# QData/FastSK

Measured on AMD Instinct MI355X. Metric: gkm kernel build: mismatch-combos/s, higher is better.
Workload: dtype u4 count planes (v_dot8_u32_u4), u32 register sums, u64 triangle (plain stores on the first pass over reset rows, else atomics); 1 GPU; config5: synthetic DNA 100000 x 300 bp, g=12 m=8 exact, 495 combos; n_seq=100000, seq_len=300, g=12, m=8, combos=495, parallelism=single GPU

## Files before the change

fastsk_amd/csrc/fsk_bytesel.h:

```cpp
#pragma once
#include "fsk_platform.h"

namespace fsk_hw {

template <int B>
__device__ __forceinline__ uint32_t add_byte(uint32_t acc, uint32_t packed) {
    static_assert(B >= 0 && B < 4, "a dword has four bytes");
#ifdef FSK_EMU
    return acc + ((packed >> (8 * B)) & 255u);
#else
    uint32_t d;
    if constexpr (B == 0)
        asm volatile("v_add_u32_sdwa %0, %1, %2 dst_sel:DWORD dst_unused:UNUSED_PAD src0_sel:BYTE_0 src1_sel:DWORD" : "=v"(d) : "v"(packed), "v"(acc));
    else if constexpr (B == 1)
        asm volatile("v_add_u32_sdwa %0, %1, %2 dst_sel:DWORD dst_unused:UNUSED_PAD src0_sel:BYTE_1 src1_sel:DWORD" : "=v"(d) : "v"(packed), "v"(acc));
    else if constexpr (B == 2)
        asm volatile("v_add_u32_sdwa %0, %1, %2 dst_sel:DWORD dst_unused:UNUSED_PAD src0_sel:BYTE_2 src1_sel:DWORD" : "=v"(d) : "v"(packed), "v"(acc));
    else
        asm volatile("v_add_u32_sdwa %0, %1, %2 dst_sel:DWORD dst_unused:UNUSED_PAD src0_sel:BYTE_3 src1_sel:DWORD" : "=v"(d) : "v"(packed), "v"(acc));
    return d;
#endif
}

template <int W>
__device__ __forceinline__ uint32_t xor_word(uint32_t packed, uint32_t x) {
    static_assert(W == 0 || W == 1, "a dword has two halves");
#ifdef FSK_EMU
    return ((packed >> (16 * W)) & 0xffffu) ^ x;
#else
    uint32_t d;
    if constexpr (W == 0)
        asm("v_xor_b32_sdwa %0, %1, %2 dst_sel:DWORD dst_unused:UNUSED_PAD src0_sel:WORD_0 src1_sel:DWORD" : "=v"(d) : "v"(packed), "v"(x));
    else
        asm("v_xor_b32_sdwa %0, %1, %2 dst_sel:DWORD dst_unused:UNUSED_PAD src0_sel:WORD_1 src1_sel:DWORD" : "=v"(d) : "v"(packed), "v"(x));
    return d;
#endif
}

__device__ __forceinline__ void first_use(uint32_t& a, uint32_t& b, uint32_t& c, uint32_t& d, uint32_t& e, uint32_t& f, uint32_t& g, uint32_t& h) {
#ifndef FSK_EMU
    asm volatile("" : "+v"(a), "+v"(b), "+v"(c), "+v"(d), "+v"(e), "+v"(f), "+v"(g), "+v"(h) : : "memory");
#endif
}

}
```

fastsk_amd/csrc/fsk_engine_dense_shift.hip:

```cpp
#include "fsk_engine_internal.h"
#include "fsk_kernels_dense_shift.h"

#include <map>

using namespace fsk_detail;

namespace fsk {

#define FSK_DMA_SHIFT 1
#define FSK_DMA_KERNEL k_dense_tile_shift
#define FSK_DMA_COMPACT 0
#include "fsk_tile_kernel_dma.inc"
#undef FSK_DMA_KERNEL
#undef FSK_DMA_SHIFT

#define FSK_DMA_SHIFT 2
#define FSK_DMA_KERNEL k_dense_tile_shift_all
#include "fsk_tile_kernel_dma.inc"
#undef FSK_DMA_KERNEL
#undef FSK_DMA_COMPACT
#undef FSK_DMA_SHIFT

}

// ... 27 lines not shown
        p.n_bases = (uint32_t)chains.size();
        p.order.resize((size_t)n);
        uint32_t derived = p.n_bases;
        size_t group_begin = 0;
        for (size_t c = 0; c < chains.size(); ++c) {
            const std::vector<int>& ch = chains[c];
            const uint32_t len = (uint32_t)ch.size();
            p.order[c] = ch[0];
            if (c == 0 || chains[c - 1].size() != ch.size() || (u64)(c - group_begin) >= by_overflow) {
                p.groups.push_back(0u);
                p.groups.push_back(len);
                group_begin = c;
            }
            p.groups[p.groups.size() - 2] = (uint32_t)c + 1u;
            uint32_t lower = (uint32_t)c;
            for (uint32_t u = 1; u < len; ++u) {
                const uint32_t upper = derived++;
                p.order[upper] = ch[u];
                p.steps.push_back(upper << 16 | lower);
                p.steps.push_back(len - u);
                p.wsum += len - u;
                lower = upper;
            }
        }
        bool falling = true;
        for (size_t gi = 2; gi + 1 < p.groups.size(); gi += 2) falling = falling && p.groups[gi + 1] < p.groups[gi - 1];
        if (falling) {
            for (size_t gi = 0; gi + 1 < p.groups.size(); gi += 2) {
                p.group_steps.push_back(p.groups[gi]);
                p.group_steps.push_back(p.groups[gi + 1] - (gi + 3 < p.groups.size() ? p.groups[gi + 3] : 0u));
            }
            p.group_steps.push_back(0xffffffffu);
            p.group_steps.push_back(0u);
        }
    }
    return !p.steps.empty() && n <= 32768 && ((u64)2 * e->maxW + 32) * p.wsum < ((u64)1 << 31);
}

static void dense_shift_unpack_flags(std::vector<uint32_t>& steps, uint32_t n_bases, bool batch) {
    const size_t n_steps = steps.size() / 2;
    uint32_t r = 0, bound = 0;
    for (size_t s = 0; s < n_steps; ++s) {
        r = (steps[2 * s] & 0xffffu) < n_bases ? 0u : r + 1u;
        const uint32_t add = 30u * (r + 1u);
        if (s > 0 && (!batch || bound + add > 255u)) {
            steps[2 * s - 1] |= 256u;
            bound = 0;
        }
        bound += add;
    }
    if (n_steps > 0) steps[2 * n_steps - 1] |= 256u;
}

int dense_shift_edge_keys(fsk_engine* e, const uint8_t* chunk_pos, uint32_t panels_pad) {
    ShiftPlan& p = e->shift;
    const uint32_t n_steps = (uint32_t)(p.steps.size() / 2), np_seq = panels_pad * fsk::PANEL;
    std::vector<uint32_t> steps = p.steps;
    dense_shift_unpack_flags(steps, p.n_bases, e->tune.dense_shift_batch != 0);
    FSK_HIP(e->d_shift_steps.reserve(p.steps.size() + p.group_steps.size()));
    FSK_HIP(e->d_edge_keys.reserve((size_t)n_steps * np_seq));
    FSK_HIP(hipMemcpyAsync(e->d_shift_steps.p, steps.data(), steps.size() * sizeof(uint32_t), hipMemcpyHostToDevice, e->stream));
    if (!p.group_steps.empty())
        FSK_HIP(hipMemcpyAsync(e->d_shift_steps.p + p.steps.size(), p.group_steps.data(), p.group_steps.size() * sizeof(uint32_t), hipMemcpyHostToDevice,
                               e->stream));
    FSK_LAUNCH(fsk::k_dense_edge_keys, dim3(panels_pad, (n_steps + 3u) / 4u), dim3(256), 0, e->stream, e->view(), e->cfg.g, e->k, e->sigma, chunk_pos,
               (const uint32_t*)e->d_shift_steps.p, n_steps, np_seq, e->d_edge_keys.p);
    FSK_HIP(hipStreamSynchronize(e->stream));
    e->st.launches += 1;
    return FSK_OK;
}

int dense_shift_keymajor(fsk_engine* e, uint32_t panels_pad, int nb, uint32_t Vq8) {
    const ShiftPlan& p = e->shift;
    e->ld.shift_packed = false;
    if (e->tune.dense_shift_packed < 0 || p.max_chain != SHIFT_PACKED_CHAIN) return FSK_OK;
    const size_t plane = (size_t)panels_pad * Vq8 * fsk::PANEL * (size_t)nb;
    const size_t n_keys = (p.steps.size() / 2) * (size_t)panels_pad * fsk::PANEL;
    const size_t want = (2 * plane + n_keys) * sizeof(uint32_t);
    const char* why = nullptr;
    if (e->tune.dense_shift_plane_kb > 0 && want > (size_t)e->tune.dense_shift_plane_kb * 1024) why = "over the dense_shift_plane_kb cap";
    const size_t grow = (std::max(plane, e->d_KM.cap) - e->d_KM.cap + std::max(plane, e->d_KMH.cap) - e->d_KMH.cap +
                         std::max(n_keys, e->d_edge_offs.cap) - e->d_edge_offs.cap) * sizeof(uint32_t);
    if (!why && grow > 0) {
        size_t free_b = 0, total_b = 0;
        if (hipMemGetInfo(&free_b, &total_b) != hipSuccess) free_b = 0;
        if (grow > free_b / 2) why = "more than half of the free device memory";
        else if (e->d_KM.reserve(plane) != hipSuccess || e->d_KMH.reserve(plane) != hipSuccess || e->d_edge_offs.reserve(n_keys) != hipSuccess) {
            (void)hipGetLastError();
            e->d_KM.release(); e->d_KMH.release(); e->d_edge_offs.release();
            why = "hipMalloc failed";
        }
    }
    if (why) {
        if (e->trace())
            fprintf(stderr, "[fsk] dense shift classes: the key-major planes (%.1f MB) do not fit, %s: k_dense_shift_fix runs the corrections\n",
                    (double)want / 1e6, why);
        return FSK_OK;
    }
    const uint32_t n_pairs = panels_pad / 2u;
    const uint32_t kgrid = (uint32_t)(((size_t)n_pairs * nb * Vq8 * 16u + 255u) / 256u);
    FSK_LAUNCH(fsk::k_dense_keymajor, dim3(kgrid), dim3(256), 0, e->stream, (const uint32_t*)e->d_C4.p, n_pairs, nb, Vq8, e->d_KM.p);
    FSK_LAUNCH(fsk::k_dense_keymajor, dim3(kgrid), dim3(256), 0, e->stream, (const uint32_t*)e->d_C4H.p, n_pairs, nb, Vq8, e->d_KMH.p);
    FSK_LAUNCH(fsk::k_dense_edge_offs, dim3((uint32_t)((n_keys + 255u) / 256u)), dim3(256), 0, e->stream, (const uint16_t*)e->d_edge_keys.p, n_keys,
               e->d_edge_offs.p);
    e->st.launches += 3;
    e->ld.shift_packed = true;
    return FSK_OK;
}

int dense_shift_tiles(fsk_engine* e, u64 n_tiles, int nb, uint32_t Vq8, uint32_t nst, u64* K, int store, uint32_t panels_pad) {
    const ShiftPlan& p = e->shift;
    const bool one_launch = !p.group_steps.empty() && (e->tune.dense_shift_one_launch > 0 ||
                                                       (e->tune.dense_shift_one_launch == 0 && e->tune.tile_splits == 0 && n_tiles >= 16384));
    int base_launches = 1;
    if (one_launch) {
        FSK_LAUNCH(fsk::k_dense_tile_shift_all, dim3((uint32_t)n_tiles, 1), dim3(256), 0, e->stream, (const uint32_t*)e->d_C4.p,
                   (const uint32_t*)e->d_C4H.p, (const uint32_t*)e->d_rowmask.p, (const uint32_t*)e->d_tiletab.p, nb, Vq8, nst, (uint32_t)e->N, K,
                   (int)p.n_bases, store, (const uint32_t*)e->d_shift_steps.p + p.steps.size());
    } else {
        base_launches = (int)(p.groups.size() / 2);
        int slot0 = 0;
        for (size_t gi = 0; gi + 1 < p.groups.size(); gi += 2) {
            const int end = (int)p.groups[gi];
            FSK_LAUNCH(fsk::k_dense_tile_shift, dim3((uint32_t)n_tiles, 1), dim3(256), 0, e->stream, (const uint32_t*)e->d_C4.p,
                       (const uint32_t*)e->d_C4H.p, (const uint32_t*)e->d_rowmask.p, (const uint32_t*)e->d_tiletab.p, nb, Vq8, nst, (uint32_t)e->N, K,
                       end - slot0, gi == 0 ? store : 0, slot0, p.groups[gi + 1]);
            slot0 = end;
        }
    }
    if (e->ld.shift_packed) {
        const auto k_packed = e->tune.dense_shift_inplace != 0 ? fsk::k_dense_shift_packed<true> : fsk::k_dense_shift_packed<false>;
        FSK_LAUNCH(k_packed, dim3((uint32_t)n_tiles), dim3(256), 0, e->stream, (const uint32_t*)e->d_KM.p, (const uint32_t*)e->d_KMH.p,
                   (const uint32_t*)e->d_rowmask.p, (const uint32_t*)e->d_tiletab.p, (const uint32_t*)e->d_shift_steps.p, (uint32_t)(p.steps.size() / 2),
                   (const uint32_t*)e->d_edge_offs.p, panels_pad * fsk::PANEL, nb, Vq8, p.n_bases, (uint32_t)(30u * p.wsum), (uint32_t)e->N, K);
    } else {
        FSK_LAUNCH(fsk::k_dense_shift_fix, dim3((uint32_t)n_tiles), dim3(512), 0, e->stream, (const uint32_t*)e->d_C4.p, (const uint32_t*)e->d_C4H.p,
                   (const uint32_t*)e->d_rowmask.p, (const uint32_t*)e->d_tiletab.p, (const uint32_t*)e->d_shift_steps.p, (uint32_t)(p.steps.size() / 2),
                   (const uint16_t*)e->d_edge_keys.p, panels_pad * fsk::PANEL, nb, Vq8, (uint32_t)e->N, K);
    }
    e->st.launches += (int32_t)base_launches;
    return FSK_OK;
}

}
```

fastsk_amd/csrc/fsk_engine_internal.h:

```cpp
#pragma once
#include "fsk_common.h"

#include <algorithm>
#include <chrono>
#include <cmath>
#include <cstdarg>
#include <cstdio>
#include <cstdlib>
#include <cstring>
#include <string>
#include <array>
#include <atomic>
#include <thread>
#include <vector>

#include <cstdint>
#include <climits>

#include "../../include/fastsk_amd.h"
#include <condition_variable>
#include <functional>
#include <memory>
#include <mutex>

// ... 50 lines not shown
        cap = 0;
    }
};

template <typename H, hipError_t (*Create)(H*, unsigned), hipError_t (*Destroy)(H)>
struct Handle {
    H h = nullptr;
    Handle() = default;
    Handle(Handle&& o) noexcept : h(o.h) { o.h = nullptr; }
    Handle& operator=(Handle&& o) noexcept { std::swap(h, o.h); return *this; }
    ~Handle() { if (h) (void)Destroy(h); }
    hipError_t create(unsigned flags) { return h ? hipSuccess : Create(&h, flags); }
    operator H() const { return h; }
};
using Stream = Handle<hipStream_t, hipStreamCreateWithFlags, hipStreamDestroy>;
using Event = Handle<hipEvent_t, hipEventCreateWithFlags, hipEventDestroy>;

struct DeviceScope {
    int prev = -1, dev;
    hipError_t err = hipSuccess;
    explicit DeviceScope(int d) : dev(d) {
        if (hipGetDevice(&prev) != hipSuccess) prev = -1;
        if (prev != dev) err = hipSetDevice(dev);
    }
    ~DeviceScope() {
        if (prev >= 0 && prev != dev) (void)hipSetDevice(prev);
    }
    DeviceScope(const DeviceScope&) = delete;
    DeviceScope& operator=(const DeviceScope&) = delete;
};
#define FSK_ON_DEVICE(e)                                                                      \
    DeviceScope fsk_on_device_((e)->cfg.device);                                             \
    if (fsk_on_device_.err != hipSuccess)                                                    \
        return (e)->fail(FSK_EDEVICE, "hipSetDevice(%d) failed: %s", (e)->cfg.device, hipGetErrorString(fsk_on_device_.err))

}

using fsk_detail::DevBuf;
using fsk_detail::PinnedBuf;
using fsk_detail::Stream;
using fsk_detail::Event;

#define FSK_TUNING_KEYS(X)                                                                                                          \
    X(trace, 0, 0, 1, "stderr: the tuning in force, where the host time of a load and of a variance-mode call goes")                 \
    X(profile, -1, -1, 2, "fsk_config.profile from here on (-1: as the engine was created)")                                          \
    X(compact, -1, -1, 1, "dense: key compaction off / on whatever the alphabet says (-1: a rare symbol decides)")                   \
    X(compact_rare, -1, -1, 1, "dense: keys that occur from the places of the rare symbols (1) or a marking pass over every window (0)") \
    X(tile_splits, 0, 0, 4096, "dense: combo splits per tile (0: by the size of the launch)")                                        \
    X(dense_small, 0, 0, 1, "dense: 1 = a split tile launch (small N) leaves its sums as 32-bit staging blocks that k_dense_widen adds into K (0: one 64-bit atomic a cell and split — measured faster: the atomics drain under other workgroups' dot products)")                                        \
    X(dense_shift, 0, -1, 1, "dense: one weighted Gram product per chain of shifted combinations, the other members by edge lookups (fsk_engine_dense_shift.hip) — 1 = whenever the call is eligible, -1 = never (0: when eligible, tile_splits = 0 and the launch has 16384 tiles or more, the size from which a tile has one workgroup anyway)") \
    X(dense_shift_packed, 0, -1, 0, "dense, shift classes: the derived steps from key-major planes, eight cells an LDS read (k_dense_keymajor, k_dense_shift_packed; chains cut at nine members) — 0 = whenever the shift path runs and the planes fit, -1 = never: k_dense_shift_fix on the count panels") \
    X(dense_shift_inplace, 1, 0, 1, "dense, shift classes: k_dense_shift_packed stages a chain's first planes and makes every further step's in LDS, one nibble up and one down a sequence (a step that meets a count above 15 in its tile, and the step behind it, are staged) — 0 = every step staged") \
    X(dense_shift_batch, 1, 0, 1, "dense, shift classes: k_dense_shift_packed adds the prefix sums of several steps byte to byte and hands the bytes to its int32 sums once a batch, where the step table says so (a step at chain position r counts 30 (r + 1) against a byte's 255; a batch may span chains) — 0 = after every step") \
    X(dense_shift_one_launch, 0, -1, 1, "dense, shift classes: every chain-length group of the base products in ONE launch that flushes at the group ends without clearing (k_dense_tile_shift_all) — 1 = whenever the shift path runs, -1 = never: one k_dense_tile_shift launch a group (0: where the shift path runs by its own default rule, tile_splits = 0 and 16384 tiles or more)") \
    X(dense_shift_plane_kb, 0, 0, (int64_t)1 << 40, "dense, shift classes: the key-major planes and offsets may take this many KiB at most (0: half of the free memory; tests: the planes do not fit)") \
    X(dense_chunk, 0, 0, 1 << 24, "dense: cap of the count kernel's staging chunk, in windows (0: none)")                             \
    X(variance_dense_slots, 1, 0, 1, "variance mode, dense: 0 = zero fill + k_welford per iteration instead of storing slot triangles") \
    X(var_slots16, 1, 0, 1, "variance mode, sparse: 0 = u32 slot triangles from the start")                                          \
    X(sparse_global, 0, 0, 1, "sparse: every += as a 64-bit atomicAdd (k_sx_emit<DIRECT>) whatever N is")                             \
    X(sparse_unpacked, 0, 0, 1, "sparse: entries in the general 8 + 4 (+ 4) byte format whatever N is")                               \
    X(sparse_pairs, 1, 0, 1, "sparse: 0 = every update word 32 bits wide (1: unit products of clean runs travel two to a word)")      \
    X(sparse_sync, 0, 0, 1, "sparse: wait for every batch's word count and size its stream exactly")                                 \
    X(sparse_hint, 1, 0, 1, "sparse: 0 = the words per record of the previous set of sequences are never kept as a hint")             \
    X(sparse_exact_lanes, 0, 0, 2, "sparse: the batches of an exact accumulate never (1) / always (2) in two lanes (0: from six batches on)") \
    X(sparse_batch_records, 0, 0, (int64_t)1 << 31, "sparse: records per batch at most (0: 2^27)")                                   \
    X(guard_cap, 0, 0, (int64_t)1 << 40, "sparse: pretend the stream buffer holds this many words (0: its real size)")                \
    X(list_max_words, 0, 0, (int64_t)1 << 31, "sparse: update words of one batch beyond which its pairs go to K with atomics (0: 2^31)") \
    X(seg_scan_chunked, 0, 0, 1, "sparse: the three-launch segment scan whatever the tile count")                                    \
    X(extract_slots, 0, 0, 4, "sparse: slots per k_sx_extract_win workgroup, 1 or 4 (0: by the size of the launch)")                  \
    X(sparse_form, 0, 0, 3, "sparse: the update stage — 1 = owner bands whenever they exist, 2 = two-level blocks, 3 = 64-bit atomics (0: bands up to four LDS rounds a band, blocks beyond)") \
    X(blocks_sub_shift, 14, 4, 14, "sparse, blocks: log2 of the cells one k_sxb_consume workgroup sums in LDS (tests: small blocks on small inputs)") \
    X(blocks_max_bands, 512, 2, 512, "sparse, blocks: bands of one pass at most (tests: several passes on small inputs)")            \
    X(blocks_band_shift_max, 23, 4, 23, "sparse, blocks: log2 of a band's cells at most (tests)")                                    \
    X(blocks_pass_words, 0, 0, (int64_t)1 << 32, "sparse, blocks: update words of one pass at most (0: 2^31)")                       \
    X(sparse_desc, 0, -1, 1, "sparse, owner bands and two-level blocks: entries of many partners leave k_sx_emit as descriptors (one an entry; blocks: one per sub-band its partners fall into) that k_sx_consume / k_sxb_consume expand in LDS — 1 = always, -1 = never (0: once a batch of these sequences has shown sparse_desc_from pairs per record)") \
    X(sparse_desc_blocks, 1, 0, 1, "sparse, two-level blocks: 0 = never descriptors there (1: as sparse_desc says — one record per sub-band an entry's partners fall into)") \
    X(sparse_desc_cols, 1, 0, 3, "sparse, descriptors: where the partners are read from — 0 = the entries themselves; 1 = a column array (sequence id | multiplicity, 4 bytes) beside 8-byte entries, the entries themselves when they are packed (measured: 2-byte columns beside packed entries are no faster, 0.88 against 0.84 s in the large-g regime; 4-byte columns beside 8-byte entries 4.69 -> 4.44 ms a combo at N = 100k); tests: 2 = 4-byte columns always, 3 = 2-byte columns when N < 32768") \
    X(sparse_desc_min, 16, 1, 48, "sparse, descriptors: entries of more partners than this become descriptors (48: everything k_sx_emit does not bin in LDS; measured, large-g regime: 48 0.92 s, 32 0.85, 16 0.83-0.85, 8 0.88, 4 0.90)") \
    X(sparse_desc_from, 12, 1, 1 << 20, "sparse, descriptors: the pairs per sort record of a batch from which on the following batches use them (sparse_desc = 0)") \
    X(sparse_parts_target, 0, 0, 1 << 30, "sparse, owner bands: words of one k_sx_consume part (0: four LDS rounds' worth at least, 1/1024 of the batch's words; tests: several parts a band on small inputs)") \
    X(sparse_desc_parts, 2048, 1, 1 << 16, "sparse, descriptors: parts (k_sx_consume workgroups) the bands' streams are cut into, about") \
    X(sparse_share, 0, -1, 254, "sparse: leading kept positions sorted once per group of consecutive combos that share them (0: by cost; -1: never); batches of more than 16 slots only (smaller ones read their positions by id), and never when the presort's scratch passes a quarter of the free memory") \
    X(seed_splitmix, 0, 0, 1, "approx modes: 1 = fsk_set_seed draws the engine's older splitmix64 Fisher-Yates order (0: the reference's std::shuffle of minstd_rand0)") \
    X(mismatch_order, 0, 0, 1, "mismatch-weighted mode: 1 = the levels run from m = d down to 0 (0: from 0 up to d)")                   \
    X(collective, 0, 0, 2, "fsk_create_multi: FSK_COLL_* when fsk_config.collective is FSK_COLL_AUTO")                                \
    X(deadline_ms, 120000, -1, 86400000, "fsk_create_multi: the fail-fast bound when fsk_config.deadline_ms is 0 (negative: none)")   \
    X(svm_wg_max, 8192, 0, 8192, "fsk_svm_train: up to this many training rows the solver is one workgroup with alpha, G and y in LDS (k_svm_wg); beyond, two launches an iteration (k_svm_select_i / k_svm_select_j); 0 = always those") \
    X(svm_chunk, 256, 1, 65536, "fsk_svm_train: iterations enqueued between two reads of the solver's status record (k_svm_wg: iterations a launch)") \
    X(rows_tile, FSK_ROWS_TILE, FSK_ROWS_TILE, FSK_ROWS_TILE, "fsk_rows_build, read-only: the edge T of k_rows_syrk's tile of the rows kernel (compiled in)") \
    X(rows_panel, FSK_ROWS_PANEL, FSK_ROWS_PANEL, FSK_ROWS_PANEL, "fsk_rows_build, read-only: the consecutive train columns P a panel of k_rows_syrk stages in LDS (compiled in)") \
    FSK_TUNING_TEST_KEYS(X)
#ifdef FSK_TEST_HOOKS
#define FSK_TUNING_TEST_KEYS(X)                                            \
    X(fault_kind, 0, 0, 3, "test hook: 1 = host sleep, 2 = device spin before a band's collective; 3 = host sleep after the variance chains")   \
    X(fault_rank, -1, -1, 15, "test hook: the engine that is late")        \
    X(fault_band, -1, -1, 63, "test hook: before this band's collective")  \
    X(fault_ms, 0, 0, 60000, "test hook: by this many milliseconds")
#else
#define FSK_TUNING_TEST_KEYS(X)
#endif
struct fsk_tuning {
#define FSK_X(name, def, lo, hi, doc) int64_t name = (def);
    FSK_TUNING_KEYS(FSK_X)
#undef FSK_X
};

// ... 71 lines not shown
    SvmCvState cv;
    SvmMcState mc, mc_cv;
    SvmMcState mc_cal;
    int model_kind = 0;
    std::vector<double> alpha;
    std::vector<double> coef;
    SvmCvState svr_cv;
    std::vector<fsk_svr_cv_score> svr_scores;
    std::vector<signed char> y;
    double rho = 0;
    int kernel = 0;
    double w_pos = 1.0, w_neg = 1.0;
    double C = 0, eps = 0;
    int64_t max_iter = 0;
    SvmCvState cal;
    bool platt_valid = false;
    fsk_svm_platt_info platt{};
    fsk_svm_info info{};
    DevBuf<double> d_alpha, d_G, d_krow, d_coef, d_out;
    DevBuf<signed char> d_y;
    DevBuf<unsigned char> d_rec;
};

struct RowsState {
    bool valid = false;
    DevBuf<double> d_L, d_diag;
    fsk_rows_info info{};
    void drop() { valid = false; d_L.release(); d_diag.release(); }
};

struct fsk_engine {
    Stream stream;
    Stream lane_stream;
    Stream chain_stream;
    fsk_config cfg{};
    int cfg_profile0 = 0;
    fsk_tuning tune{};
    std::string err;
    int k = 0;
    int64_t ncomb = 0;
    Event ev0, ev1;
    Event ev_out, ev_in;
    fsk_group* group = nullptr;
    bool store_next = false;
    PinnedBuf<uint32_t> h_stage;
    bool stage_in_flight = false;
    PinnedBuf<double> h_prod;

    struct Loaded {
        bool featseq_ready = false;
        bool rare_ready = false;
        bool prep_valid = false, prep_overflow = false, prep_shift = false, shift_packed = false;
        uint32_t prep_chain = 0;
        double vc_sum = 0, vc_n = 0;
        bool u_known = false, u_pending = false;
        u64 u_value = 0, u_extra = 0;
        struct SxDefer { bool active = false; u64 cap = 0, nrec = 0; } sx_defer[8];
        int64_t lazy_lo = -1, lazy_hi = -1;
        std::vector<double> stdevs;
        u64 sx_passes = 0;
        int sx_form_used = -1;
        bool sx_desc_used = false;
        int sx_share_used = 0;
        uint32_t sx_share_groups = 0;
    } ld;

    bool loaded = false, finalized = false, result_f64 = false;
    int64_t N = 0, n_train = 0, n_test = 0, nfeat = 0, pairs = 0;
    uint32_t sigma = 0, Lmax = 0, Lmin = 0, maxW = 0, Vq = 0, n_panels = 0;
    int bits = 0;
    u64 V = 0;
    int path = 0;
    DevBuf<uint32_t> d_words, d_wstart, d_len, d_fstart, d_featseq;
    DevBuf<uint32_t> d_win;
    int win_words = 0;
    std::vector<uint32_t> h_len, h_fstart;
    std::vector<int32_t> rc_tokens, rc_comps;
    bool revcomp = false;
    uint32_t maxW1 = 0;
    DevBuf<uint16_t> d_comp;
    std::vector<int32_t> wild_tokens;
    bool wild = false;
    DevBuf<uint32_t> d_vbits, d_vstart, d_fwin;
    std::vector<uint8_t> cw_profile;
    bool cw = false, fwin_on = false;
    uint32_t cw_n = 0;
    DevBuf<uint8_t> d_cw;

    std::vector<uint64_t> mm_c;
    std::vector<int64_t> mm_a;
    bool mm_plain = false;
    DevBuf<u64> mm_scratch;
    std::vector<int64_t> mm_ran_a;
    std::vector<int32_t> mm_ran_path;
    std::vector<double> mm_ran_level_ms, mm_ran_fold_ms;
    bool mm_on() const { return !mm_c.empty(); }

    std::vector<uint8_t> all_pos;
    DevBuf<uint8_t> d_pos, d_allpos;
    bool allpos_ready = false;
    std::vector<int32_t> order;
    bool order_set = false;
    uint64_t seed = 0;

    u64* d_K = nullptr;
    bool K_owned = false;
// ... 230 lines not shown
```

fastsk_amd/csrc/fsk_kernels_dense_shift.h:

```cpp
#pragma once
#include "fsk_bytesel.h"
#include "fsk_common.h"

namespace fsk {

__device__ __forceinline__ uint32_t panel_seq(uint32_t p) { return (p >> 2) + 16u * (p & 3u); }

__global__ __launch_bounds__(256) void k_dense_edge_keys(SeqView S, int g, int k, uint32_t sigma, const uint8_t* combo_pos, const uint32_t* steps,
                                                         uint32_t n_steps, uint32_t np_seq, uint16_t* keys) {
    const uint32_t r = threadIdx.x & 63u, step = blockIdx.y * 4u + (threadIdx.x >> 6), panel = blockIdx.x;
    if (step >= n_steps) return;
    const uint32_t seq = panel * PANEL + r;
    const uint32_t sl = steps[2u * step], up = sl >> 16, lo = sl & 0xffffu;
    uint32_t kd = 0, ks = 0;
    if (seq < S.n_seq) {
        const uint32_t len = S.len[seq], wbase = S.wstart[seq];
        if (len >= (uint32_t)g) {
            const uint32_t last = len - (uint32_t)g;
            for (int c = 0; c < k; ++c) {
                kd = kd * sigma + fetch_sym(S.words, wbase, (uint32_t)combo_pos[(size_t)lo * k + c], S.bits);
                ks = ks * sigma + fetch_sym(S.words, wbase, last + (uint32_t)combo_pos[(size_t)up * k + c], S.bits);
            }
        }
    }
// ... 109 lines not shown
        for (int q = 0; q < QW; ++q) {
            const uint32_t i = (uint32_t)h * PANEL + lane, j = w * (uint32_t)QW + (uint32_t)q;
            T[i * TILE + ((j + i) & (TILE - 1u))] = accR[h][q];
        }
    __syncthreads();
#pragma unroll
    for (int h = 0; h < 2; ++h) {
        const uint32_t jd = (uint32_t)h * PANEL + lane;
        const u64 j = (u64)tj * TILE + (uint32_t)h * PANEL + panel_seq(lane);
#pragma unroll
        for (int q = 0; q < QW; ++q) {
            const uint32_t id = w * (uint32_t)QW + (uint32_t)q;
            const u64 i = (u64)ti * TILE + (id >> 6) * PANEL + panel_seq(id & 63u);
            const int v = accC[h][q] + T[id * TILE + ((jd + id) & (TILE - 1u))];
            if (i < N && j <= i && v != 0) atomicAdd(&K[tri_index(i, j)], (u64)(long long)v);
        }
    }
}

__device__ __forceinline__ uint32_t km_swizzle(uint32_t key) { return ((key >> 1) & 3u) << 2; }
__device__ __forceinline__ uint32_t km_offset(uint32_t key) { return key << 6 | km_swizzle(key) << 2; }

__global__ __launch_bounds__(256) void k_dense_keymajor(const uint32_t* plane, uint32_t n_pairs, int n_slots, uint32_t Vq8, uint32_t* KM) {
    const size_t id = (size_t)blockIdx.x * 256u + threadIdx.x;
    const uint32_t t = (uint32_t)id & 15u;
    size_t rest = id >> 4;
    const uint32_t row = (uint32_t)(rest % Vq8);
    rest /= Vq8;
    const uint32_t slot = (uint32_t)(rest % (uint32_t)n_slots);
    const size_t pair = rest / (uint32_t)n_slots;
    if (pair >= n_pairs) return;
    const size_t slot_stride = (size_t)Vq8 * PANEL, panel_stride = (size_t)n_slots * slot_stride;
    const uint32_t* src = plane + 2u * pair * panel_stride + slot * slot_stride + (size_t)row * PANEL + 4u * t;
    const uint4 a = *reinterpret_cast<const uint4*>(src), b = *reinterpret_cast<const uint4*>(src + panel_stride);
    const uint32_t in[8] = {a.x, a.y, a.z, a.w, b.x, b.y, b.z, b.w};
    uint32_t* out = KM + (pair * (size_t)n_slots + slot) * ((size_t)Vq8 * 128u);
#pragma unroll
    for (uint32_t q = 0; q < 8u; ++q) {
        uint32_t v = 0;
#pragma unroll
        for (uint32_t n = 0; n < 8u; ++n) v |= ((in[n] >> (4u * q)) & 15u) << (4u * n);
        const uint32_t key = row * 8u + q;
        out[key * 16u + (t ^ km_swizzle(key))] = v;
    }
}

__global__ __launch_bounds__(256) void k_dense_edge_offs(const uint16_t* keys, size_t n, uint32_t* offs) {
    const size_t q = (size_t)blockIdx.x * 256u + threadIdx.x;
    if (q >= n) return;
    const uint32_t kk = keys[q];
    offs[q] = km_offset(kk & 255u) | km_offset(kk >> 8) << 16;
}

template <bool INPLACE>
__global__ __launch_bounds__(256, 2) void k_dense_shift_packed(const uint32_t* KM, const uint32_t* KMH, const uint32_t* rowmask, const uint32_t* tile_tab,
                                                               const uint32_t* steps, uint32_t n_steps, const uint32_t* offs, uint32_t np_seq,
                                                               int n_slots, uint32_t Vq8, uint32_t n_bases, uint32_t bias, uint32_t N, u64* K) {
    constexpr uint32_t SIDE = 256u * 16u;
    constexpr uint32_t PBUF = 2u * SIDE;
    __shared__ __attribute__((aligned(1024))) uint32_t P[2 * PBUF];
    const uint32_t tid = threadIdx.x, lane = tid & 63u;
    const uint32_t w = (uint32_t)__builtin_amdgcn_readfirstlane(tid >> 6);
    const uint32_t M4 = (uint32_t)__builtin_amdgcn_readfirstlane(fsk_hw::vgpr_copy(0x0f0f0f0fu));
    const uint32_t tr = (w >> 1) * 8u + (lane >> 3), tc = (w & 1u) * 8u + (lane & 7u);
    const uint32_t tile = tile_tab[blockIdx.x];
    const uint32_t ti = tile >> 16, tj = tile & 0xffffu;
    const size_t slot_stride = (size_t)Vq8 * 128u;
    const size_t pair_stride = (size_t)n_slots * slot_stride;
    const uint32_t side_bytes = Vq8 * 512u;

    uint32_t acc[8][8], Rr[2][8], Rc[2][8], Qr[2][8], Qc[2][8];
#pragma unroll
    for (int a = 0; a < 8; ++a) {
#pragma unroll
        for (int b = 0; b < 8; ++b) acc[a][b] = 0u;
        Rr[0][a] = Rr[1][a] = Rc[0][a] = Rc[1][a] = 0u;
        Qr[0][a] = Qr[1][a] = Qc[0][a] = Qc[1][a] = 0u;
    }

    const fsk_hw::lds_addr_t lds_wave = fsk_hw::lds_address(P) + w * 1024u;
    auto load_stage = [&](const uint32_t* plane, uint32_t buf, uint32_t sl) {
        const uint32_t up = sl >> 16, lo = sl & 0xffffu;
#pragma unroll
        for (uint32_t side = 0; side < 2u; ++side) {
            const uint32_t* src = plane + (side == 0u ? ti : tj) * pair_stride + (size_t)(side == 0u ? up : lo) * slot_stride;
#pragma unroll
            for (uint32_t q = 0; q < 4u; ++q)
                if (q * 4096u < side_bytes)
                    fsk_hw::panel_rows_to_lds(src, side_bytes, lds_wave + (buf * PBUF + side * SIDE + q * 1024u) * 4u, q * 4096u + tid * 16u);
        }
    };
    auto load_offs = [&](uint32_t s, uint4 (&oR)[2], uint4 (&oC)[2]) {
        const uint32_t* os = offs + (size_t)s * np_seq;
#pragma unroll
        for (uint32_t h = 0; h < 2u; ++h) {
            oR[h] = *reinterpret_cast<const uint4*>(os + ti * TILE + h * PANEL + 4u * tr);
            oC[h] = *reinterpret_cast<const uint4*>(os + tj * TILE + h * PANEL + 4u * tc);
        }
    };
    auto flagged = [&](uint32_t sl) {
        const uint32_t up = sl >> 16, lo = sl & 0xffffu;
        const uint32_t mA = rowmask[(size_t)(ti * 2u) * n_slots + up] | rowmask[(size_t)(ti * 2u + 1u) * n_slots + up];
        const uint32_t mB = rowmask[(size_t)(tj * 2u) * n_slots + lo] | rowmask[(size_t)(tj * 2u + 1u) * n_slots + lo];
        return mA | mB;
    };
    auto lds_at = [&](uint32_t byte_off) { return *reinterpret_cast<const uint32_t*>(reinterpret_cast<const char*>(P) + byte_off); };

    uint32_t sl = steps[0], wt = steps[1], fl = flagged(sl);
    uint32_t sn = n_steps > 1u ? steps[2] : 0u, wn = n_steps > 1u ? steps[3] : 0u;
    uint32_t s2 = 0u, w2 = 0u, fl_nx = 0u;
    if constexpr (INPLACE) {
        if (n_steps > 2u) { s2 = steps[4]; w2 = steps[5]; }
        if (n_steps > 1u) fl_nx = flagged(sn);
    }
    uint4 oR_n[2], oC_n[2];
    load_offs(0u, oR_n, oC_n);
    uint32_t buf = 0;
    load_stage(KM, 0u, sl);
    fsk_hw::wait_panel_rows();
    __syncthreads();
    for (uint32_t s = 0; s < n_steps; ++s) {
        uint32_t oR[8], oC[8];
#pragma unroll
        for (int h = 0; h < 2; ++h) {
            oR[4 * h] = fsk_hw::vgpr_copy(oR_n[h].x); oR[4 * h + 1] = fsk_hw::vgpr_copy(oR_n[h].y);
            oR[4 * h + 2] = fsk_hw::vgpr_copy(oR_n[h].z); oR[4 * h + 3] = fsk_hw::vgpr_copy(oR_n[h].w);
            oC[4 * h] = fsk_hw::vgpr_copy(oC_n[h].x); oC[4 * h + 1] = fsk_hw::vgpr_copy(oC_n[h].y);
            oC[4 * h + 2] = fsk_hw::vgpr_copy(oC_n[h].z); oC[4 * h + 3] = fsk_hw::vgpr_copy(oC_n[h].w);
        }
        const bool same = INPLACE && s + 1u < n_steps && (sn & 0xffffu) >= n_bases && fl == 0u && fl_nx == 0u;
        uint32_t uo_n = 0u;
        if (s + 1u < n_steps) {
            load_offs(s + 1u, oR_n, oC_n);
            if (same) uo_n = offs[(size_t)(w < 2u ? s + 1u : s) * np_seq + (w < 2u ? ti : tj) * TILE + (tid & 127u)];
            else load_stage(KM, buf ^ 1u, sn);
        }
        if ((sl & 0xffffu) < n_bases) {
#pragma unroll
            for (int a = 0; a < 8; ++a) Rr[0][a] = Rr[1][a] = Rc[0][a] = Rc[1][a] = 0u;
        }
        const uint32_t baseA = buf * PBUF * 4u, baseB = baseA + SIDE * 4u;
        const uint32_t xA = (tr * 4u) | baseA, xB = (tc * 4u) | baseB;
        uint32_t dA[8], sA[8], dB[8], sB[8];
        auto read_A = [&](int e) { dA[e] = lds_at(fsk_hw::xor_word<0>(oC[e], xA)); sA[e] = lds_at(fsk_hw::xor_word<1>(oC[e], xA)); };
        auto read_B = [&](int e) { dB[e] = lds_at(fsk_hw::xor_word<0>(oR[e], xB)); sB[e] = lds_at(fsk_hw::xor_word<1>(oR[e], xB)); };
        auto row_term = [&](int e) {
            Rr[0][e] += (sA[e] & M4) + (~dA[e] & M4);
            Rr[1][e] += ((sA[e] >> 4) & M4) + (~(dA[e] >> 4) & M4);
            Qr[0][e] += Rr[0][e];
            Qr[1][e] += Rr[1][e];
        };
        auto col_term = [&](int e) {
            Rc[0][e] += (sB[e] & M4) + (~dB[e] & M4);
            Rc[1][e] += ((sB[e] >> 4) & M4) + (~(dB[e] >> 4) & M4);
            Qc[0][e] += Rc[0][e];
            Qc[1][e] += Rc[1][e];
        };
#pragma unroll
        for (int e = 0; e < 8; ++e) read_A(e);
        fsk_hw::first_use(dA[0], sA[0], dA[1], sA[1], dA[2], sA[2], dA[3], sA[3]);
#pragma unroll
        for (int e = 0; e < 4; ++e) read_B(e);
#pragma unroll
        for (int e = 0; e < 4; ++e) row_term(e);
        fsk_hw::first_use(dA[4], sA[4], dA[5], sA[5], dA[6], sA[6], dA[7], sA[7]);
#pragma unroll
        for (int e = 4; e < 8; ++e) read_B(e);
#pragma unroll
        for (int e = 4; e < 8; ++e) row_term(e);
        fsk_hw::first_use(dB[0], sB[0], dB[1], sB[1], dB[2], sB[2], dB[3], sB[3]);
#pragma unroll
        for (int e = 0; e < 4; ++e) col_term(e);
        fsk_hw::first_use(dB[4], sB[4], dB[5], sB[5], dB[6], sB[6], dB[7], sB[7]);
#pragma unroll
        for (int e = 4; e < 8; ++e) col_term(e);
        if ((wt & 256u) != 0u) {
#pragma unroll
            for (int e = 0; e < 8; ++e) {
                acc[0][e] = fsk_hw::add_byte<0>(acc[0][e], Qr[0][e]); acc[1][e] = fsk_hw::add_byte<0>(acc[1][e], Qr[1][e]);
                acc[2][e] = fsk_hw::add_byte<1>(acc[2][e], Qr[0][e]); acc[3][e] = fsk_hw::add_byte<1>(acc[3][e], Qr[1][e]);
                acc[4][e] = fsk_hw::add_byte<2>(acc[4][e], Qr[0][e]); acc[5][e] = fsk_hw::add_byte<2>(acc[5][e], Qr[1][e]);
                acc[6][e] = fsk_hw::add_byte<3>(acc[6][e], Qr[0][e]); acc[7][e] = fsk_hw::add_byte<3>(acc[7][e], Qr[1][e]);
            }
#pragma unroll
            for (int e = 0; e < 8; ++e) {
                acc[e][0] = fsk_hw::add_byte<0>(acc[e][0], Qc[0][e]); acc[e][1] = fsk_hw::add_byte<0>(acc[e][1], Qc[1][e]);
                acc[e][2] = fsk_hw::add_byte<1>(acc[e][2], Qc[0][e]); acc[e][3] = fsk_hw::add_byte<1>(acc[e][3], Qc[1][e]);
                acc[e][4] = fsk_hw::add_byte<2>(acc[e][4], Qc[0][e]); acc[e][5] = fsk_hw::add_byte<2>(acc[e][5], Qc[1][e]);
                acc[e][6] = fsk_hw::add_byte<3>(acc[e][6], Qc[0][e]); acc[e][7] = fsk_hw::add_byte<3>(acc[e][7], Qc[1][e]);
                Qr[0][e] = Qr[1][e] = Qc[0][e] = Qc[1][e] = 0u;
            }
        }
        if (fl != 0u) {
            __syncthreads();
            load_stage(KMH, buf, sl);
            fsk_hw::wait_panel_rows();
            __syncthreads();
            const uint32_t mul = 16u * (wt & 255u);
#pragma unroll
            for (int e = 0; e < 8; ++e) {
                read_A(e);
                read_B(e);
#pragma unroll
                for (int n = 0; n < 8; ++n) {
                    acc[n][e] += (((sA[e] >> (4 * n)) & 15u) - ((dA[e] >> (4 * n)) & 15u)) * mul;
                    acc[e][n] += (((sB[e] >> (4 * n)) & 15u) - ((dB[e] >> (4 * n)) & 15u)) * mul;
                }
            }
        }
        uint32_t fl_n = 0u, sl_n2 = 0u, wt_n2 = 0u;
        if constexpr (INPLACE) {
            if (s + 2u < n_steps) {
                fl_n = flagged(s2);
                if (s + 3u < n_steps) {
                    sl_n2 = steps[2u * (s + 3u)];
                    wt_n2 = steps[2u * (s + 3u) + 1u];
                }
            }
        } else if (s + 1u < n_steps) {
            fl_n = flagged(sn);
            if (s + 2u < n_steps) {
                sl_n2 = steps[2u * (s + 2u)];
                wt_n2 = steps[2u * (s + 2u) + 1u];
            }
        }
        fsk_hw::wait_panel_rows();
        __syncthreads();
        if (same) {
            const uint32_t uo = fsk_hw::vgpr_copy(uo_n), od = uo & 0xffffu, os = uo >> 16;
            if (od != os) {
                const uint32_t p = tid & 127u, t4 = p & 0x3cu, e = (p >> 6) * 4u + (p & 3u);
                const uint32_t base = buf * PBUF + (w >> 1) * SIDE, inc = 1u << (4u * e);
                atomicAdd(&P[base + ((os ^ t4) >> 2)], inc);
                atomicAdd(&P[base + ((od ^ t4) >> 2)], 0u - inc);
            }
            __syncthreads();
        } else {
            buf ^= 1u;
        }
        if constexpr (INPLACE) {
            sl = sn; wt = wn; fl = fl_nx;
            sn = s2; wn = w2; fl_nx = fl_n;
            s2 = sl_n2; w2 = wt_n2;
        } else {
            sl = sn; wt = wn; fl = fl_n;
            sn = sl_n2; wn = wt_n2;
        }
    }
#pragma unroll
    for (int er = 0; er < 8; ++er) {
        const u64 i = (u64)ti * TILE + tile_index(tr, (uint32_t)er);
#pragma unroll
        for (int ec = 0; ec < 8; ++ec) {
            const u64 j = (u64)tj * TILE + tile_index(tc, (uint32_t)ec);
            const int v = (int)(acc[er][ec] - bias);
            if (i < N && j <= i && v != 0) atomicAdd(&K[tri_index(i, j)], (u64)(long long)v);
        }
    }
}

}
```

Baseline: 464.1 combos/s.

## Stage next chain's planes and key offsets ahead at chain start in LDS

Adds an AHEAD variant of the packed shift kernel. A host-built chain table describes each chain, and at a chain's first step the kernel stages the next chain's first planes into the idle buffer and its key offsets into an LDS ring, so steps inside a chain issue no vector memory loads. In-chain barriers become LDS-only waits (lgkmcnt plus s_barrier) instead of full waits. The cost is larger LDS use per workgroup (about 80 KB), which may reduce occupancy below the two workgroups the launch bounds ask for, plus more complex control flow with a fallback path for flagged chains.

```diff
diff --git a/fastsk_amd/csrc/fsk_bytesel.h b/fastsk_amd/csrc/fsk_bytesel.h
--- a/fastsk_amd/csrc/fsk_bytesel.h
+++ b/fastsk_amd/csrc/fsk_bytesel.h
@@ -43,4 +43,12 @@
 #endif
 }
 
+__device__ __forceinline__ void barrier_lds_only() {
+#ifdef FSK_EMU
+    __syncthreads();
+#else
+    asm volatile("s_waitcnt lgkmcnt(0)\n\ts_barrier" ::: "memory");
+#endif
 }
+
+}
diff --git a/fastsk_amd/csrc/fsk_engine_dense_shift.hip b/fastsk_amd/csrc/fsk_engine_dense_shift.hip
--- a/fastsk_amd/csrc/fsk_engine_dense_shift.hip
+++ b/fastsk_amd/csrc/fsk_engine_dense_shift.hip
@@ -103,17 +103,43 @@
     if (n_steps > 0) steps[2 * n_steps - 1] |= 256u;
 }
 
+static std::vector<uint32_t> dense_shift_chain_table(const std::vector<uint32_t>& steps, uint32_t n_bases) {
+    std::vector<uint32_t> t;
+    const size_t n_steps = steps.size() / 2;
+    size_t s = 0;
+    while (s < n_steps) {
+        const uint32_t sl0 = steps[2 * s], up0 = sl0 >> 16, wt0 = steps[2 * s + 1] & 255u;
+        if ((sl0 & 0xffffu) >= n_bases) return {};
+        uint32_t len = 0, flags = 0;
+        for (; s + len < n_steps && (len == 0 || (steps[2 * (s + len)] & 0xffffu) >= n_bases); ++len) {
+            const uint32_t sl = steps[2 * (s + len)], wt = steps[2 * (s + len) + 1];
+            if (len > 0 && sl != ((up0 + len) << 16 | (up0 + len - 1u))) return {};
+            if (len >= 8 || wt0 < len || (wt & 255u) != wt0 - len || up0 + len > 0xffffu) return {};
+            flags |= ((wt >> 8) & 1u) << len;
+        }
+        t.push_back(sl0);
+        t.push_back(len | wt0 << 8 | flags << 16);
+        s += len;
+    }
+    return t;
+}
+
 int dense_shift_edge_keys(fsk_engine* e, const uint8_t* chunk_pos, uint32_t panels_pad) {
     ShiftPlan& p = e->shift;
     const uint32_t n_steps = (uint32_t)(p.steps.size() / 2), np_seq = panels_pad * fsk::PANEL;
     std::vector<uint32_t> steps = p.steps;
     dense_shift_unpack_flags(steps, p.n_bases, e->tune.dense_shift_batch != 0);
-    FSK_HIP(e->d_shift_steps.reserve(p.steps.size() + p.group_steps.size()));
+    const std::vector<uint32_t> chain_tab = dense_shift_chain_table(steps, p.n_bases);
+    FSK_HIP(e->d_shift_steps.reserve(p.steps.size() + p.group_steps.size() + chain_tab.size()));
     FSK_HIP(e->d_edge_keys.reserve((size_t)n_steps * np_seq));
     FSK_HIP(hipMemcpyAsync(e->d_shift_steps.p, steps.data(), steps.size() * sizeof(uint32_t), hipMemcpyHostToDevice, e->stream));
     if (!p.group_steps.empty())
         FSK_HIP(hipMemcpyAsync(e->d_shift_steps.p + p.steps.size(), p.group_steps.data(), p.group_steps.size() * sizeof(uint32_t), hipMemcpyHostToDevice,
                                e->stream));
+    if (!chain_tab.empty())
+        FSK_HIP(hipMemcpyAsync(e->d_shift_steps.p + p.steps.size() + p.group_steps.size(), chain_tab.data(), chain_tab.size() * sizeof(uint32_t),
+                               hipMemcpyHostToDevice, e->stream));
+    e->ld.shift_chains = (uint32_t)(chain_tab.size() / 2);
     FSK_LAUNCH(fsk::k_dense_edge_keys, dim3(panels_pad, (n_steps + 3u) / 4u), dim3(256), 0, e->stream, e->view(), e->cfg.g, e->k, e->sigma, chunk_pos,
                (const uint32_t*)e->d_shift_steps.p, n_steps, np_seq, e->d_edge_keys.p);
     FSK_HIP(hipStreamSynchronize(e->stream));
@@ -180,10 +206,13 @@
         }
     }
     if (e->ld.shift_packed) {
-        const auto k_packed = e->tune.dense_shift_inplace != 0 ? fsk::k_dense_shift_packed<true> : fsk::k_dense_shift_packed<false>;
+        const bool ahead = e->tune.dense_shift_inplace != 0 && e->tune.dense_shift_ahead != 0 && e->ld.shift_chains > 0;
+        const auto k_packed = ahead ? fsk::k_dense_shift_packed<true, true>
+                                    : e->tune.dense_shift_inplace != 0 ? fsk::k_dense_shift_packed<true, false> : fsk::k_dense_shift_packed<false, false>;
         FSK_LAUNCH(k_packed, dim3((uint32_t)n_tiles), dim3(256), 0, e->stream, (const uint32_t*)e->d_KM.p, (const uint32_t*)e->d_KMH.p,
-                   (const uint32_t*)e->d_rowmask.p, (const uint32_t*)e->d_tiletab.p, (const uint32_t*)e->d_shift_steps.p, (uint32_t)(p.steps.size() / 2),
-                   (const uint32_t*)e->d_edge_offs.p, panels_pad * fsk::PANEL, nb, Vq8, p.n_bases, (uint32_t)(30u * p.wsum), (uint32_t)e->N, K);
+                   (const uint32_t*)e->d_rowmask.p, (const uint32_t*)e->d_tiletab.p,
+                   (const uint32_t*)e->d_shift_steps.p + (ahead ? p.steps.size() + p.group_steps.size() : 0), (uint32_t)(p.steps.size() / 2),
+                   (const uint32_t*)e->d_edge_offs.p, panels_pad * fsk::PANEL, nb, Vq8, ahead ? e->ld.shift_chains : p.n_bases, (uint32_t)(30u * p.wsum), (uint32_t)e->N, K);
     } else {
         FSK_LAUNCH(fsk::k_dense_shift_fix, dim3((uint32_t)n_tiles), dim3(512), 0, e->stream, (const uint32_t*)e->d_C4.p, (const uint32_t*)e->d_C4H.p,
                    (const uint32_t*)e->d_rowmask.p, (const uint32_t*)e->d_tiletab.p, (const uint32_t*)e->d_shift_steps.p, (uint32_t)(p.steps.size() / 2),
diff --git a/fastsk_amd/csrc/fsk_engine_internal.h b/fastsk_amd/csrc/fsk_engine_internal.h
--- a/fastsk_amd/csrc/fsk_engine_internal.h
+++ b/fastsk_amd/csrc/fsk_engine_internal.h
@@ -126,6 +126,7 @@
     X(dense_shift_packed, 0, -1, 0, "dense, shift classes: the derived steps from key-major planes, eight cells an LDS read (k_dense_keymajor, k_dense_shift_packed; chains cut at nine members) — 0 = whenever the shift path runs and the planes fit, -1 = never: k_dense_shift_fix on the count panels") \
     X(dense_shift_inplace, 1, 0, 1, "dense, shift classes: k_dense_shift_packed stages a chain's first planes and makes every further step's in LDS, one nibble up and one down a sequence (a step that meets a count above 15 in its tile, and the step behind it, are staged) — 0 = every step staged") \
     X(dense_shift_batch, 1, 0, 1, "dense, shift classes: k_dense_shift_packed adds the prefix sums of several steps byte to byte and hands the bytes to its int32 sums once a batch, where the step table says so (a step at chain position r counts 30 (r + 1) against a byte's 255; a batch may span chains) — 0 = after every step") \
+    X(dense_shift_ahead, 1, 0, 1, "dense, shift classes: k_dense_shift_packed stages the NEXT chain's first planes and key offsets at a chain's first step, into the idle stage buffer and an offsets ring in LDS (80 KB a workgroup), and issues no vector memory load inside a chain (a chain that meets a count above 15 in its tile stages as before) — 0 = every chain start staged one step ahead; ignored with dense_shift_inplace = 0 and on the k_dense_shift_fix path") \
     X(dense_shift_one_launch, 0, -1, 1, "dense, shift classes: every chain-length group of the base products in ONE launch that flushes at the group ends without clearing (k_dense_tile_shift_all) — 1 = whenever the shift path runs, -1 = never: one k_dense_tile_shift launch a group (0: where the shift path runs by its own default rule, tile_splits = 0 and 16384 tiles or more)") \
     X(dense_shift_plane_kb, 0, 0, (int64_t)1 << 40, "dense, shift classes: the key-major planes and offsets may take this many KiB at most (0: half of the free memory; tests: the planes do not fit)") \
     X(dense_chunk, 0, 0, 1 << 24, "dense: cap of the count kernel's staging chunk, in windows (0: none)")                             \
@@ -303,6 +304,7 @@
         bool rare_ready = false;
         bool prep_valid = false, prep_overflow = false, prep_shift = false, shift_packed = false;
         uint32_t prep_chain = 0;
+        uint32_t shift_chains = 0;
         double vc_sum = 0, vc_n = 0;
         bool u_known = false, u_pending = false;
         u64 u_value = 0, u_extra = 0;
diff --git a/fastsk_amd/csrc/fsk_kernels_dense_shift.h b/fastsk_amd/csrc/fsk_kernels_dense_shift.h
--- a/fastsk_amd/csrc/fsk_kernels_dense_shift.h
+++ b/fastsk_amd/csrc/fsk_kernels_dense_shift.h
@@ -185,13 +185,15 @@
     offs[q] = km_offset(kk & 255u) | km_offset(kk >> 8) << 16;
 }
 
-template <bool INPLACE>
+template <bool INPLACE, bool AHEAD = false>
 __global__ __launch_bounds__(256, 2) void k_dense_shift_packed(const uint32_t* KM, const uint32_t* KMH, const uint32_t* rowmask, const uint32_t* tile_tab,
                                                                const uint32_t* steps, uint32_t n_steps, const uint32_t* offs, uint32_t np_seq,
                                                                int n_slots, uint32_t Vq8, uint32_t n_bases, uint32_t bias, uint32_t N, u64* K) {
+    static_assert(INPLACE || !AHEAD, "the ahead schedule is a schedule of the in-place form");
     constexpr uint32_t SIDE = 256u * 16u;
     constexpr uint32_t PBUF = 2u * SIDE;
-    __shared__ __attribute__((aligned(1024))) uint32_t P[2 * PBUF];
+    constexpr uint32_t RING = 8u * 256u;
+    __shared__ __attribute__((aligned(1024))) uint32_t P[AHEAD ? 2 * PBUF + 2 * RING : 2 * PBUF];
     const uint32_t tid = threadIdx.x, lane = tid & 63u;
     const uint32_t w = (uint32_t)__builtin_amdgcn_readfirstlane(tid >> 6);
     const uint32_t M4 = (uint32_t)__builtin_amdgcn_readfirstlane(fsk_hw::vgpr_copy(0x0f0f0f0fu));
@@ -239,19 +241,82 @@
     };
     auto lds_at = [&](uint32_t byte_off) { return *reinterpret_cast<const uint32_t*>(reinterpret_cast<const char*>(P) + byte_off); };
 
-    uint32_t sl = steps[0], wt = steps[1], fl = flagged(sl);
-    uint32_t sn = n_steps > 1u ? steps[2] : 0u, wn = n_steps > 1u ? steps[3] : 0u;
+    uint32_t sl, wt, fl, sn = 0u, wn = 0u;
     uint32_t s2 = 0u, w2 = 0u, fl_nx = 0u;
-    if constexpr (INPLACE) {
-        if (n_steps > 2u) { s2 = steps[4]; w2 = steps[5]; }
-        if (n_steps > 1u) fl_nx = flagged(sn);
-    }
     uint4 oR_n[2], oC_n[2];
-    load_offs(0u, oR_n, oC_n);
     uint32_t buf = 0;
-    load_stage(KM, 0u, sl);
-    fsk_hw::wait_panel_rows();
-    __syncthreads();
+    [[maybe_unused]] uint32_t* const ring = P + 2u * PBUF;
+    [[maybe_unused]] uint32_t cb = 0u, dv0 = 0u, dv1 = 0u;
+    [[maybe_unused]] uint32_t c = 0u, r = 0u, rem = 0u;
+    [[maybe_unused]] uint32_t n0 = 0u, n1 = 0u, mk_n = 0u;
+    [[maybe_unused]] uint32_t flw = 0u, wu = 0u, slq = 0u;
+    [[maybe_unused]] uint32_t half = 0u, rg = 0u;
+    [[maybe_unused]] bool lost = false;
+    [[maybe_unused]] auto enter_chain = [&](uint32_t e0, uint32_t e1, uint32_t mk) {
+        flw = (uint32_t)__ballot(fsk_hw::vgpr_copy(mk) != 0u);
+        sl = e0;
+        slq = ((e0 >> 16) + 1u) << 16 | (e0 >> 16);
+        rem = e1 & 15u;
+        wt = (e1 >> 8) & 255u;
+        wu = e1 >> 16;
+        r = 0u;
+        rg = half * RING;
+    };
+    [[maybe_unused]] auto load_desc = [&]() {
+        const uint32_t q = cb + lane < n_bases ? cb + lane : n_bases - 1u;
+        dv0 = steps[2u * q];
+        dv1 = steps[2u * q + 1u];
+    };
+    [[maybe_unused]] auto load_masks = [&](uint32_t e0, uint32_t e1) {
+        const uint32_t mr = lane >> 2, x = lane & 3u, up0 = e0 >> 16;
+        uint32_t m = 0u;
+        if (mr < (e1 & 15u)) {
+            const uint32_t slot = x < 2u ? up0 + mr : (mr == 0u ? (e0 & 0xffffu) : up0 + mr - 1u);
+            m = rowmask[(size_t)((x < 2u ? ti : tj) * 2u + (x & 1u)) * n_slots + slot];
+        }
+        return m;
+    };
+    [[maybe_unused]] auto load_ring = [&](uint32_t hf, uint32_t s_first, uint32_t n) {
+        const uint32_t ring_lane = lane < 32u ? (ti * TILE + 4u * lane) * 4u : (tj * TILE + 4u * (lane - 32u)) * 4u;
+#pragma unroll
+        for (uint32_t q = 0; q < 2u; ++q) {
+            const uint32_t rr = w + 4u * q;
+            if (rr < n)
+                fsk_hw::panel_rows_to_lds(offs + (size_t)(s_first + rr) * np_seq, np_seq * 4u, fsk_hw::lds_address(ring) + (hf * RING + rr * 256u) * 4u,
+                                          ring_lane);
+        }
+    };
+    [[maybe_unused]] auto ring_offs = [&](uint32_t at, uint4 (&oR)[2], uint4 (&oC)[2]) {
+        const uint32_t* q = ring + at;
+#pragma unroll
+        for (uint32_t hh = 0; hh < 2u; ++hh) {
+            oR[hh] = *reinterpret_cast<const uint4*>(q + hh * PANEL + 4u * tr);
+            oC[hh] = *reinterpret_cast<const uint4*>(q + TILE + hh * PANEL + 4u * tc);
+        }
+    };
+    if constexpr (AHEAD) {
+        load_desc();
+        const uint32_t d0 = fsk_hw::readlane(dv0, 0u), d1 = fsk_hw::readlane(dv1, 0u);
+        const uint32_t mk = load_masks(d0, d1);
+        load_stage(KM, 0u, d0);
+        load_ring(0u, 0u, d1 & 15u);
+        fsk_hw::wait_panel_rows();
+        __syncthreads();
+        fl = 0u;
+        enter_chain(d0, d1, mk);
+        ring_offs(0u, oR_n, oC_n);
+    } else {
+        sl = steps[0]; wt = steps[1]; fl = flagged(sl);
+        sn = n_steps > 1u ? steps[2] : 0u; wn = n_steps > 1u ? steps[3] : 0u;
+        if constexpr (INPLACE) {
+            if (n_steps > 2u) { s2 = steps[4]; w2 = steps[5]; }
+            if (n_steps > 1u) fl_nx = flagged(sn);
+        }
+        load_offs(0u, oR_n, oC_n);
+        load_stage(KM, 0u, sl);
+        fsk_hw::wait_panel_rows();
+        __syncthreads();
+    }
     for (uint32_t s = 0; s < n_steps; ++s) {
         uint32_t oR[8], oC[8];
 #pragma unroll
@@ -261,14 +326,53 @@
             oC[4 * h] = fsk_hw::vgpr_copy(oC_n[h].x); oC[4 * h + 1] = fsk_hw::vgpr_copy(oC_n[h].y);
             oC[4 * h + 2] = fsk_hw::vgpr_copy(oC_n[h].z); oC[4 * h + 3] = fsk_hw::vgpr_copy(oC_n[h].w);
         }
-        const bool same = INPLACE && s + 1u < n_steps && (sn & 0xffffu) >= n_bases && fl == 0u && fl_nx == 0u;
+        bool same;
         uint32_t uo_n = 0u;
-        if (s + 1u < n_steps) {
-            load_offs(s + 1u, oR_n, oC_n);
-            if (same) uo_n = offs[(size_t)(w < 2u ? s + 1u : s) * np_seq + (w < 2u ? ti : tj) * TILE + (tid & 127u)];
-            else load_stage(KM, buf ^ 1u, sn);
-        }
-        if ((sl & 0xffffu) < n_bases) {
+        [[maybe_unused]] bool last = false;
+        if constexpr (AHEAD) {
+            const bool first = r == 0u, has_next = c + 1u < n_bases;
+            last = rem == 1u;
+            if (first) {
+                lost = false;
+                if (has_next) {
+                    if (c + 1u - cb >= 64u) {
+                        cb = c;
+                        load_desc();
+                    }
+                    n0 = fsk_hw::readlane(dv0, c + 1u - cb);
+                    n1 = fsk_hw::readlane(dv1, c + 1u - cb);
+                    mk_n = load_masks(n0, n1);
+                }
+            }
+            fl = flw & 15u;
+            wt = (wt & 255u) | (wu & 1u) << 8;
+            same = !last && (flw & 255u) == 0u;
+            if (first && has_next) {
+                if (last || same) load_stage(KM, buf ^ 1u, n0);
+                else lost = true;
+                load_ring(half ^ 1u, s + rem, n1 & 15u);
+            }
+            if (!last) {
+                ring_offs(rg + 256u, oR_n, oC_n);
+                if (same) {
+                    uo_n = ring[rg + (w < 2u ? 256u : (uint32_t)TILE) + (tid & 127u)];
+                } else {
+                    lost = true;
+                    if (!first) fsk_hw::wait_panel_rows();
+                    load_stage(KM, buf ^ 1u, slq);
+                }
+            } else if (lost && has_next) {
+                load_stage(KM, buf ^ 1u, n0);
+            }
+        } else {
+            same = INPLACE && s + 1u < n_steps && (sn & 0xffffu) >= n_bases && fl == 0u && fl_nx == 0u;
+            if (s + 1u < n_steps) {
+                load_offs(s + 1u, oR_n, oC_n);
+                if (same) uo_n = offs[(size_t)(w < 2u ? s + 1u : s) * np_seq + (w < 2u ? ti : tj) * TILE + (tid & 127u)];
+                else load_stage(KM, buf ^ 1u, sn);
+            }
+        }
+        if (AHEAD ? r == 0u : (sl & 0xffffu) < n_bases) {
 #pragma unroll
             for (int a = 0; a < 8; ++a) Rr[0][a] = Rr[1][a] = Rc[0][a] = Rc[1][a] = 0u;
         }
@@ -341,43 +445,76 @@
                 }
             }
         }
-        uint32_t fl_n = 0u, sl_n2 = 0u, wt_n2 = 0u;
-        if constexpr (INPLACE) {
-            if (s + 2u < n_steps) {
-                fl_n = flagged(s2);
-                if (s + 3u < n_steps) {
-                    sl_n2 = steps[2u * (s + 3u)];
-                    wt_n2 = steps[2u * (s + 3u) + 1u];
-                }
-            }
-        } else if (s + 1u < n_steps) {
-            fl_n = flagged(sn);
-            if (s + 2u < n_steps) {
-                sl_n2 = steps[2u * (s + 2u)];
-                wt_n2 = steps[2u * (s + 2u) + 1u];
-            }
-        }
-        fsk_hw::wait_panel_rows();
-        __syncthreads();
-        if (same) {
-            const uint32_t uo = fsk_hw::vgpr_copy(uo_n), od = uo & 0xffffu, os = uo >> 16;
-            if (od != os) {
-                const uint32_t p = tid & 127u, t4 = p & 0x3cu, e = (p >> 6) * 4u + (p & 3u);
-                const uint32_t base = buf * PBUF + (w >> 1) * SIDE, inc = 1u << (4u * e);
-                atomicAdd(&P[base + ((os ^ t4) >> 2)], inc);
-                atomicAdd(&P[base + ((od ^ t4) >> 2)], 0u - inc);
-            }
+        if constexpr (AHEAD) {
+            if (last) {
+                fsk_hw::wait_panel_rows();
+                __syncthreads();
+                buf ^= 1u;
+                if (c + 1u < n_bases) {
+                    half ^= 1u;
+                    enter_chain(n0, n1, mk_n);
+                    ring_offs(rg, oR_n, oC_n);
+                }
+                ++c;
+            } else {
+                if (same) {
+                    fsk_hw::barrier_lds_only();
+                    const uint32_t uo = fsk_hw::vgpr_copy(uo_n), od = uo & 0xffffu, os = uo >> 16;
+                    if (od != os) {
+                        const uint32_t p = tid & 127u, t4 = p & 0x3cu, e = (p >> 6) * 4u + (p & 3u);
+                        const uint32_t base = buf * PBUF + (w >> 1) * SIDE, inc = 1u << (4u * e);
+                        atomicAdd(&P[base + ((os ^ t4) >> 2)], inc);
+                        atomicAdd(&P[base + ((od ^ t4) >> 2)], 0u - inc);
+                    }
+                    fsk_hw::barrier_lds_only();
+                } else {
+                    fsk_hw::wait_panel_rows();
+                    __syncthreads();
+                    buf ^= 1u;
+                }
+                sl = slq; slq += 0x10001u;
+                --rem; --wt; wu >>= 1; flw >>= 4;
+                ++r; rg += 256u;
+            }
+        } else {
+            uint32_t fl_n = 0u, sl_n2 = 0u, wt_n2 = 0u;
+            if constexpr (INPLACE) {
+                if (s + 2u < n_steps) {
+                    fl_n = flagged(s2);
+                    if (s + 3u < n_steps) {
+                        sl_n2 = steps[2u * (s + 3u)];
+                        wt_n2 = steps[2u * (s + 3u) + 1u];
+                    }
+                }
+            } else if (s + 1u < n_steps) {
+                fl_n = flagged(sn);
+                if (s + 2u < n_steps) {
+                    sl_n2 = steps[2u * (s + 2u)];
+                    wt_n2 = steps[2u * (s + 2u) + 1u];
+                }
+            }
+            fsk_hw::wait_panel_rows();
             __syncthreads();
-        } else {
-            buf ^= 1u;
-        }
-        if constexpr (INPLACE) {
-            sl = sn; wt = wn; fl = fl_nx;
-            sn = s2; wn = w2; fl_nx = fl_n;
-            s2 = sl_n2; w2 = wt_n2;
-        } else {
-            sl = sn; wt = wn; fl = fl_n;
-            sn = sl_n2; wn = wt_n2;
+            if (same) {
+                const uint32_t uo = fsk_hw::vgpr_copy(uo_n), od = uo & 0xffffu, os = uo >> 16;
+                if (od != os) {
+                    const uint32_t p = tid & 127u, t4 = p & 0x3cu, e = (p >> 6) * 4u + (p & 3u);
+                    const uint32_t base = buf * PBUF + (w >> 1) * SIDE, inc = 1u << (4u * e);
+                    atomicAdd(&P[base + ((os ^ t4) >> 2)], inc);
+                    atomicAdd(&P[base + ((od ^ t4) >> 2)], 0u - inc);
+                }
+                __syncthreads();
+            } else {
+                buf ^= 1u;
+            }
+            if constexpr (INPLACE) {
+                sl = sn; wt = wn; fl = fl_nx;
+                sn = s2; wn = w2; fl_nx = fl_n;
+                s2 = sl_n2; w2 = wt_n2;
+            } else {
+                sl = sn; wt = wn; fl = fl_n;
+                sn = sl_n2; wn = wt_n2;
+            }
         }
     }
 #pragma unroll
```

New measurement: 472.2 combos/s, median of 6. 1.02x the previous value.
